# utiasDSL/upright

Hardware: AMD Instinct MI355X
Metric: batched MPC solves/sec + ms/SQP-iter, Thing 1-obj horizon=20, 1/2/4/8 GPU (higher is better)
Workload: dtype f64

## Files before the change

__graft_entry__.py:

```python
import os
import subprocess
import sys
from pathlib import Path

ROOT = Path(__file__).resolve().parent
CSRC = ROOT / "upright_amd" / "csrc"
LIB = ROOT / "upright_amd" / "libupright_mi.so"


def _newer(srcs, out):
    return (not out.exists()) or any(s.stat().st_mtime > out.stat().st_mtime for s in srcs)


def n_qp3_parts():
    import re

    m = re.search(r"#define\s+UPR_QP3_NPARTS\s+(\d+)", (CSRC / "upr_qp3_list.h").read_text())
    return int(m.group(1))


def build_engine(out=None, extra_flags=()):
    from concurrent.futures import ThreadPoolExecutor

    out = Path(out) if out else LIB
    hipcc = os.environ.get("HIPCC", "/opt/rocm/bin/hipcc")
    flags = ["--offload-arch=gfx950", "-O3", "-std=c++17", "-fPIC", "-Wno-unused-value", "-Wno-pass-failed", *extra_flags]
    obj = CSRC / "build"
    obj.mkdir(exist_ok=True)
    jobs = [([hipcc, *flags, "-c", str(CSRC / "upr_api.hip"), "-o", str(obj / "upr_api.o")], obj / "upr_api.o")]
    for k in range(n_qp3_parts()):
        o = obj / f"upr_qp3_part{k}.o"
        jobs.append(([hipcc, *flags, f"-DUPR_QP3_PART={k}", "-c", str(CSRC / "upr_qp3_inst.hip"), "-o", str(o)], o))
    with ThreadPoolExecutor(max_workers=max(1, min(len(jobs), os.cpu_count() or 1))) as ex:
        for rc, cmd in ex.map(lambda j: (subprocess.call(j[0]), j[0]), jobs):
            if rc != 0:
                raise subprocess.CalledProcessError(rc, cmd)
    subprocess.check_call([hipcc, "--offload-arch=gfx950", "-shared", "-fPIC", "-o", str(out), *[str(o) for _, o in jobs], "-lhiprtc", "-ldl"])


def build():
    srcs = sorted(CSRC.glob("*.h")) + sorted(CSRC.glob("*.hip")) + [ROOT / "include" / "upright_mi.h"]
    if _newer(srcs, LIB):
        build_engine()
    subprocess.check_call(["make", "-s", "-C", str(ROOT / "oracle")])
    emu_src = ROOT / "tests" / "emu" / "upr_emu.cpp"
    emu_out = ROOT / "tests" / "emu" / "libupr_emu.so"
    if _newer(srcs + [emu_src], emu_out):
        subprocess.check_call(["g++", "-O2", "-std=c++17", "-fPIC", "-shared", "-Wno-unknown-pragmas", "-o", str(emu_out), str(emu_src)])
    vf_src = ROOT / "tests" / "emu" / "upr_vf_emu.cpp"
    vf_out = ROOT / "tests" / "emu" / "libupr_vf_emu.so"
    if _newer(srcs + [vf_src], vf_out):
        subprocess.check_call(["g++", "-O2", "-std=c++17", "-fPIC", "-shared", "-Wno-unknown-pragmas", "-o", str(vf_out), str(vf_src)])
    sys.path.insert(0, str(ROOT))
    import upright_amd
    from upright_amd import _capi

    _capi.lib()


def smoke():
    import json

    import numpy as np

    sys.path.insert(0, str(ROOT))
    from oracle.oracle import Oracle
    from upright_amd.engine import BatchMPC
    from upright_amd.problem import thing_problem
    from upright_amd.sampling import level_tray_states, stationary_guess, waypoints_for

    arr = json.load(open(ROOT / "tests" / "golden" / "arrangements.json"))["pink_bottle"]
    P = thing_problem(arr)
    B = 4
    x0 = level_tray_states(B, seed=3)
    way = waypoints_for(P, x0)
    mpc = BatchMPC(P, B, way_p=way)
    mpc.set_observation(0.0, x0)
    mpc.advance()
    _, xs, us = mpc.solution()
    st = mpc.stats()
    xs0, us0 = stationary_guess(x0, P.N, P.nu)
    for b in range(B):
        P.way_p = way[b]
        xo, uo, so, _ = Oracle(P).solve(0.0, x0[b], xs0[b], us0[b])
        ex, eu = np.abs(xo - xs[b]).max(), np.abs(uo - us[b]).max()
        assert ex < 1e-4 and eu < 1e-4 * max(1.0, np.abs(uo).max()), (b, ex, eu)
        assert abs(np.linalg.norm(xo) - np.linalg.norm(xs[b])) < 1e-4
        assert abs(np.linalg.norm(uo) - np.linalg.norm(us[b])) < 1e-4
    print("smoke ok: qp iters", st["qp_iters_last"], "cost", st["cost"])


if __name__ == "__main__":
    build()
    if len(sys.argv) > 1 and sys.argv[1] == "smoke":
        smoke()
```

upright_amd/csrc/upr_qp3.h:

```cpp
#pragma once
#include "upr_kin.h"
#include "upr_qp.h"
#include "upr_qp2.h"

#ifndef UPR_QP3_INCEK
#define UPR_QP3_INCEK 1
#endif
#ifndef UPR_QP3_GQ
#define UPR_QP3_GQ 5
#endif
#ifndef UPR_QP3_SOFT_ROWMEM
#define UPR_QP3_SOFT_ROWMEM 1
#endif
template <int NQ_, int NB_, int NC_, int NF_, int N_, int NT_, bool ROWS_ = true, bool SOFT_ = false, bool DENSE_ = false>
struct upr_qp3_cfg {
    static constexpr int NQ = NQ_, NB = NB_, NC = NC_, NF = NF_, N = N_, NT = NT_;
    static constexpr bool ROWS = ROWS_, SOFT = SOFT_, COUPLED = DENSE_ && NB_ > 1, MULTI = NB_ > 1 && !DENSE_;
    static constexpr bool INCEK = UPR_QP3_INCEK && NB_ > 1 && !DENSE_ && NF_ == 1;
    static constexpr bool BIGF = MULTI && NF_ == 3;
    static constexpr bool KFAR = N_ > 64;
    static_assert(!KFAR || (MULTI && !BIGF && !ROWS_), "long horizons: star arrangements without friction and without state-polytopic rows (the upright_robust shape)");
    static constexpr int SB = COUPLED ? 6 * NB_ : 6, NKB = COUPLED ? N_ : N_ * NB_;
    static constexpr int NLS = COUPLED ? 36 * NB_ * NB_ : NB_ * 36;
    static constexpr int N1 = N + 1;
    static constexpr int NX = 3 * NQ, NFC = NF * NC, NU = NQ + NFC, NE = 6 * NB;
    static constexpr int NP = (NF == 3) ? 5 * NC : 0;
    static constexpr int NLF = (NF == 3) ? 9 * NC : NC;
    static constexpr int NH = NQ * (NQ + 1) / 2;
    static constexpr int NZ = N1 * NX + N * NU;
    static constexpr int NEN = 3 + 2 * NQ;
    static constexpr bool SW = NH <= 64 && 4 * NQ <= 64;
    static constexpr bool VCPRE = SW && NB_ == 1;
    static constexpr int NXI = N * NX, QX = (NXI + NT - 1) / NT;
    static constexpr int NUI = N * NU, QU = (NUI + NT - 1) / NT;
    static constexpr int NCI = N * NC, QC = (NCI + NT - 1) / NT;
    static constexpr int SS_V = 0, SS_LJI = SS_V + NQ * NX, SS_YJ = SS_LJI + NQ * NQ, SS_PB = SS_YJ + NQ, SS_STRIDE = ((SS_PB + NX + 1) & ~1);
};

#ifndef UPR_QP3_NOMAX
#define UPR_QP3_NOMAX 20
#endif
template <class C>
struct upr_qp3_far {
    static constexpr int r2(int n) { return (n + 1) & ~1; }
    static constexpr int g0 = 0, e0 = g0 + r2(C::N * C::NQ), ek = e0 + r2(C::N * C::NE), yf = ek + r2(C::N * C::NE), hf = yf + r2(C::N * C::NFC),
                         ys = hf + r2(C::N * C::NFC), zt = ys + r2(C::N * C::NE), cv = zt, nun = zt + r2(C::N * C::NE), lfi = nun + r2(C::N * C::NE),
                         Ljis = lfi + r2(C::N * C::NLF), ct = Ljis + r2(C::N * (C::SW ? C::NQ * C::NX : C::NH)),
                          cl = ct + r2(5 * C::NCI), cc = cl + r2(5 * C::NCI),
                         hee = cc + r2(5 * C::NCI), lsi = hee + r2(C::N * C::NH), Ks = lsi + r2(C::N * C::NLS),
                         cxr = Ks + r2(C::N * C::NQ * C::NX), rows = cxr + r2((C::SOFT ? 2 : 1) * (2 * C::QX + 2 * C::QU) * C::NT),
                         ot = rows + r2((C::SOFT ? 10 : 4) * (C::QX + C::QU) * C::NT), ol = ot + (C::N - 1) * UPR_QP3_NOMAX, oc = ol + (C::N - 1) * UPR_QP3_NOMAX,
                         od0 = oc + (C::N - 1) * UPR_QP3_NOMAX, heew = od0 + (C::N - 1) * UPR_QP3_NOMAX,
                         sfr = heew + r2(C::N * C::NH), sor = sfr + (C::SOFT ? 4 * r2(5 * C::NCI) : 0),
                         total = sor + ((C::SOFT && C::ROWS) ? 4 * (C::N - 1) * UPR_QP3_NOMAX : 0);
    static constexpr int sfs = r2(5 * C::NCI), sos = (C::N - 1) * UPR_QP3_NOMAX;
};

template <class C>
struct upr_qp3_lds {
    static constexpr int r2(int n) { return (n + 1) & ~1; }
    static constexpr bool KF = C::KFAR;
    static constexpr int Z = 0, S = Z + r2(C::NZ), gxs = S + r2(C::NZ), wx = gxs + r2(C::N1 * C::NX), gus = wx + r2(C::N1 * C::NX),
                         wu = gus + r2(C::N * C::NU), cs = wu + r2(C::N * C::NU), hf = cs + r2(C::N * C::NX), ys = hf + r2(C::BIGF ? 0 : C::N * C::NFC),
                         zt = ys + r2(C::N * C::NE), cv = zt, ek = zt + r2(C::N * C::NE),
                         dek = ek + r2(C::BIGF ? 0 : C::N * C::NE),
                         kend = dek + r2(C::INCEK ? C::N * C::NE : 0),
                         xlb = KF ? 0 : kend, xub = xlb + r2(C::NX), ulb = xub + r2(C::NX), uub = ulb + r2(C::NU), qd = uub + r2(C::NU),
                         rd = qd + r2(C::NX), xd = rd + r2(C::NU), erow = xd + r2(C::NX), df = erow + r2(3 * (C::NP > 0 ? C::NP : 1)),
                         Pa = df + r2(C::BIGF ? 6 * C::NFC : C::NE * C::NFC), Pb = Pa + r2(C::NX * C::NX), hux = Pb + r2(C::NX * C::NX),
                         vm = hux + r2(C::NQ * C::NX), lk = vm + 2 * r2(C::NQ * C::NX),
                         hjj = lk + 2 * r2(C::NH), vc = hjj + r2(C::NQ * C::NQ), ck = vc + r2(C::NE * C::NX),
                         VCS = (C::NE * 2 % 64 == 32 || C::NE * 2 % 64 == 0) ? C::NE + 2 : C::NE ,
                         VCN = VCS * C::NX, KS = (r2(C::NZ) / VCN < C::N - 1) ? r2(C::NZ) / VCN : C::N - 1, HXS = (C::NQ + 1) & ~1,
                         sw0 = C::VCPRE ? Pa + (C::N - 1 - KS) * VCN : Pa, sw_vcb = sw0 ,
                         sw_hj = C::VCPRE ? sw0 : sw0 + 2 * VCN, sw_hx = sw_hj + r2(C::NH), sw_pb = sw_hx + (C::NX + C::NQ) * HXS , sw_w = sw_pb + C::NX * HXS ,
                         sw_pq = sw_w + r2(C::NX) ,
                         sw_end = sw_pq + (C::VCPRE ? 0 : 2 * 9 * 64),
                         scr_sweep = ck + r2(C::NE * C::NX), scr_sw = C::SW ? ((KF || sw_end > sw0 + C::NKB * (C::SB * (C::SB + 1) / 2)) ? sw_end : sw0 + r2(C::NKB * (C::SB * (C::SB + 1) / 2))) : 0,
                         sst = (C::MULTI || C::COUPLED) ? hux : (Pa + r2(C::N * C::NE * C::NFC) > hux ? Pa + r2(C::N * C::NE * C::NFC) : hux),
                         scr_prep = sst + r2((C::MULTI || C::COUPLED) ? 0 : C::N * C::NE * C::NE), scr_rows = hux + (C::ROWS ? 2 * (C::N - 1) * UPR_QP3_NOMAX : 0),
                         scr_a = scr_sweep > scr_sw ? scr_sweep : scr_sw, scr_b = scr_prep > scr_rows ? scr_prep : scr_rows,
                         yN = scr_a > scr_b ? scr_a : scr_b, dyN = yN + r2(C::NEN),
                         eN = dyN + r2(C::NEN), jN = eN + r2(C::NEN), red = jN + r2(3 * C::NQ), RSET = (4 * (C::NT / 64) > 16 ? 4 * (C::NT / 64) : 16) , misc = red + 2 * RSET,
                         prf = misc + 16, lsik = prf + 4 * 16,    heek = lsik + r2(C::NLS), lend = heek + 2 * r2(C::NH), Pbs = KF ? kend : lend, kffs = Pbs + r2(C::N * C::NX),
                         bks = kffs + r2(C::N * C::NQ), gee = bks + r2(C::N * C::NX),
                         kend2 = gee + r2(C::N * C::NQ), clist = KF ? lend : kend2, ccnt = clist + r2(C::NB > 1 ? C::NB * C::NC : 0),
                         sdn = ccnt + r2(C::NB > 1 ? C::NB : 0),
                         plist = sdn + r2(C::COUPLED ? C::N * (C::SB * (C::SB + 1) / 2) : 0), pcnt = plist + r2(C::COUPLED ? (C::NB * (C::NB + 1) / 2) * C::NC : 0),
                         total = pcnt + r2(C::COUPLED ? C::NB * (C::NB + 1) / 2 : 0),
                         zst = KF ? kend2 : Pa, pin = KF ? zst + r2(C::N * C::NFC * 6) : Pa, ktotal = KF ? pin + r2(C::N1 * C::NX) : 0;
};

template <class C>
struct upr_qp3_ws {
    static constexpr int dx = 0, du = C::N1 * C::NX;
    static constexpr int a0 = (C::NZ + 1) & ~1;
    static constexpr int pi = a0, pin = pi + C::N1 * C::NX + (C::N1 * C::NX & 1), nu = pin + C::N1 * C::NX + (C::N1 * C::NX & 1),
                         store = nu + ((C::N * C::NE + 1) & ~1), far = store , kfar = far + upr_qp3_far<C>::total , total = ((kfar + upr_qp3_lds<C>::ktotal + 15) & ~15);
};

#ifndef UPR_QP3_KSTAGES
#define UPR_QP3_KSTAGES 6
#endif
#ifndef UPR_QP3_PRIO
#define UPR_QP3_PRIO 1
#endif
#ifndef UPR_QP3_PRIO_W0
#define UPR_QP3_PRIO_W0 3
#endif
#ifndef UPR_QP3_PRIO_VEC
#define UPR_QP3_PRIO_VEC 3
#endif
#ifndef UPR_QP3_PRIO_FWD
#define UPR_QP3_PRIO_FWD 3
#endif
#ifndef UPR_QP3_PRIO_W1
#define UPR_QP3_PRIO_W1 (C::SOFT ? 3 : 1)
#endif
#ifndef UPR_QP3_OCC1
#define UPR_QP3_OCC1 2
#endif
#ifndef UPR_QP3_PREC_MAX
#define UPR_QP3_PREC_MAX 4
#endif
#ifndef UPR_QP3_PREV_MAX
#define UPR_QP3_PREV_MAX 8
#endif
#if defined(UPR_HOST_EMU) || !UPR_QP3_PRIO
#define UPR_SETPRIO(p) ((void)0)
#else
#define UPR_SETPRIO(p) __builtin_amdgcn_s_setprio(p)
#endif
template <class C>
#define UPR_FORT(i, n) for (int i = tid(); i < (n); i += stride())

struct upr_qp3 {
    typedef upr_qp3_lds<C> O;
    typedef upr_qp3_ws<C> W;
    typedef upr_qp3_far<C> F;
    static constexpr int NQ = C::NQ, NX = C::NX, NU = C::NU, NE = C::NE, NFC = C::NFC, NC = C::NC, NF = C::NF, N = C::N, N1 = C::N1, NT = C::NT;
#ifndef UPR_HOST_EMU
    static constexpr bool SW2 = C::SW;
    static_assert(!C::SW || NT >= 128, "the two-wave matrix sweep needs two waves");
#else
    static constexpr bool SW2 = false;
#endif
    UPR_HDI static void sync_lds() { if (C::KFAR) { UPR_SYNC(); } else { UPR_SYNC_LDS(); } }
    UPR_HDI static void wsync_lds() { if (C::KFAR) { UPR_WSYNC(); } else { UPR_WSYNC_LDS(); } }
    upr_ctx ctx;
    int wb;
    UPR_HDI int lane() const {
#ifdef UPR_HOST_EMU
        return ctx.tid;
#else
        int z; asm volatile("s_mov_b32 %0, 0" : "=s"(z));
        return (int)__builtin_amdgcn_mbcnt_hi(~0u, __builtin_amdgcn_mbcnt_lo(~0u, (unsigned)z));
#endif
    }
    UPR_HDI int tid() const {
#ifdef UPR_HOST_EMU
        return ctx.tid;
#else
        return wb + lane();
#endif
    }
    UPR_HDI bool wave0() const {
#ifdef UPR_HOST_EMU
        return ctx.tid < 64;
#else
        return wb == 0;
#endif
    }
    UPR_HDI int stride() const {
// ... 1451 lines not shown
    UPR_HDI void backward_mat() {
#ifndef UPR_HOST_EMU
        static_assert(C::SW, "device instantiations run the two-wave matrix sweep (chains of up to nine joints)");
        backward_mat_sw2();
#else
#include "upr_qp3_emu_mat.h"
#endif
    }

    UPR_HDI double* Wk(int k) const { return LK + O::S + (k + 1) * NX; }
    UPR_HDI void backward_vec(bool fused = false) {
        const double irho = 1.0 / UPR_QP_RHO_N;
        if (!fused) {
        terminal_residual();
        UPR_SYNC();
        }
        toc(11);
        if (!fused && wave0()) {
            UPR_SETPRIO(UPR_QP3_PRIO_VEC);
            UPR_FORT(i, NX) {
                double v = LK[O::gxs + N * NX + i];
                if (neN > 0) {
                    if (i < NQ) { for (int q = 0; q < 3; ++q) v -= L[O::jN + q * NQ + i] * (L[O::yN + q] + irho * L[O::eN + q]); }
                    else v += L[O::yN + 3 + (i - NQ)] + irho * L[O::eN + 3 + (i - NQ)];
                }
                Wk(N - 1)[i] = v + LK[O::Pbs + (N - 1) * NX + i];
            }
            UPR_WSYNC();
#ifndef UPR_HOST_EMU
            static_assert(4 * NQ <= 64, "one quad per joint");
            {
                const int l = lane();
                const bool act = ((l & 3) < 3) && ((l >> 2) < NQ);
                const int j = act ? (l >> 2) : 0, b = act ? (l & 3) : 0;
                const int i = b * NQ + j;
                double kc[UPR_QP3_KSTAGES][NQ];
#define UPR_LOADKC(dst, kk) do { if (act && (kk) >= 1) { _Pragma("unroll") for (int m = 0; m < NQ; ++m) dst[m] = G[F::Ks + (kk) * NQ * NX + m * NX + i]; } } while (0)
#define UPR_LOADST(gk, pk, uk, kk) do { if ((kk) >= 1) { gk = LK[O::gxs + (kk) * NX + i] + LK[O::cs + (kk) * NX + i]; pk = LK[O::Pbs + ((kk) - 1) * NX + i]; uk = LK[O::gus + (kk) * NU + j]; } } while (0)
#define UPR_VECSTEP(kcx, gk, pk, uk, kk) do { \
                    double rq = cbq * wv; \
                    rq += upr_dpp_quad<0xB1>(rq); rq += upr_dpp_quad<0x4E>(rq); \
                    rq += uk; \
                    const double w0 = upr_dpp_quad<0x00>(wv), w1 = upr_dpp_quad<0x55>(wv), w2 = upr_dpp_quad<0xAA>(wv); \
                    double v0 = gk + ca0 * w0, v1 = ca1 * w1, v2 = ca2 * w2; \
                    _Pragma("unroll") for (int m = 0; m < NQ; m += 3) { \
                        v0 -= kcx[m] * upr_readlane(rq, 4 * m); \
                        if (m + 1 < NQ) v1 -= kcx[m + 1] * upr_readlane(rq, 4 * (m + 1)); \
                        if (m + 2 < NQ) v2 -= kcx[m + 2] * upr_readlane(rq, 4 * (m + 2)); } \
                    wv = ((v0 + v1) + v2) + pk; \
                    if (act) Wk((kk) - 1)[i] = wv; } while (0)
                const double ca0 = coefA(0, b), ca1 = (b >= 1) ? coefA(1, b) : 0.0, ca2 = (b >= 2) ? 1.0 : 0.0;
                const double cbq = act ? coefB(b) : 0.0;
#pragma unroll
                for (int st = 0; st < UPR_QP3_KSTAGES; ++st) {
#pragma unroll
                    for (int m = 0; m < NQ; ++m) kc[st][m] = 0.0;
                    UPR_LOADKC(kc[st], N - 1 - st);
                }
                double wv = Wk(N - 1)[i];
                double gs[2] = {0.0, 0.0}, ps[2] = {0.0, 0.0}, us2[2] = {0.0, 0.0};
                UPR_LOADST(gs[(N - 1) & 1], ps[(N - 1) & 1], us2[(N - 1) & 1], N - 1);
                constexpr int UG = C::KFAR ? UPR_QP3_KSTAGES : N - 1;
                static_assert(!C::KFAR || UPR_QP3_KSTAGES % 2 == 0, "the two operand slots keep their parity over a group");
#pragma unroll 1
                for (int k0 = N - 1; k0 >= 1; k0 -= UG) {
#pragma unroll
                    for (int sg = 0; sg < UG; ++sg) {
                        const int k = k0 - sg;
                        if (k >= 1) {
                            UPR_LOADST(gs[(N - sg) & 1], ps[(N - sg) & 1], us2[(N - sg) & 1], k - 1);
                            UPR_VECSTEP(kc[sg % UPR_QP3_KSTAGES], gs[(N - 1 - sg) & 1], ps[(N - 1 - sg) & 1], us2[(N - 1 - sg) & 1], k);
                            UPR_LOADKC(kc[sg % UPR_QP3_KSTAGES], k - UPR_QP3_KSTAGES);
                        }
                    }
                }
#undef UPR_LOADKC
#undef UPR_LOADST
#undef UPR_VECSTEP
            }
#else
            for (int k = N - 1; k >= 1; --k) {
                const double* w = Wk(k);
                UPR_FORT(i, NX) {
                    const int b = i / NQ, j = i % NQ;
                    double v = LK[O::gxs + k * NX + i] + LK[O::cs + k * NX + i];
                    for (int a = 0; a <= b; ++a) v += coefA(a, b) * w[a * NQ + j];
                    for (int m = 0; m < NQ; ++m) v -= G[F::Ks + k * NQ * NX + m * NX + i] * (LK[O::gus + k * NU + m] + h3 * w[m] + h2 * w[NQ + m] + h * w[2 * NQ + m]);
                    Wk(k - 1)[i] = v + LK[O::Pbs + (k - 1) * NX + i];
                }
            }
#endif
            UPR_SETPRIO(0);
        }
#ifndef UPR_HOST_EMU
        constexpr bool KFFW1 = SW2 && N <= 64 && NT >= 128;
        const bool kfw = KFFW1 && !fused;
        double liP[KFFW1 ? NQ : 1][KFFW1 ? NQ : 1];
        if (kfw && wb == 64) {
            const int k = (lane() < N) ? lane() : 0;
            const double* Li = G + F::Ljis + k * NQ * NX;
#pragma unroll
            for (int i = 0; i < NQ; ++i)
#pragma unroll
                for (int m = 0; m <= i; ++m) liP[i % (KFFW1 ? NQ : 1)][m % (KFFW1 ? NQ : 1)] = Li[i * NX + m];
        }
#endif
        UPR_SYNC();
        toc(10);
#ifndef UPR_HOST_EMU
        if constexpr (SW2) {
            for (int k = kfw ? tid() - 64 : tid(); k >= 0 && k < N; k += kfw ? N : stride()) {
                const double* Li = G + F::Ljis + k * NQ * NX;
                const double* w = Wk(k);
                double li[NQ][NQ], tv[NQ], y[NQ];
#pragma unroll
                for (int i = 0; i < NQ; ++i)
#pragma unroll
                    for (int m = 0; m <= i; ++m) li[i][m] = kfw ? liP[i % (KFFW1 ? NQ : 1)][m % (KFFW1 ? NQ : 1)] : Li[i * NX + m];
#pragma unroll
                for (int i = 0; i < NQ; ++i) tv[i] = fused ? LK[O::kffs + k * NQ + i] : LK[O::gus + k * NU + i] + h3 * w[i] + h2 * w[NQ + i] + h * w[2 * NQ + i];
#pragma unroll
                for (int i = 0; i < NQ; ++i) { double t = 0.0;
#pragma unroll
                    for (int m = 0; m <= i; ++m) t += li[i][m] * tv[m];
                    y[i] = t; }
#pragma unroll
                for (int i = 0; i < NQ; ++i) { double t = 0.0;
#pragma unroll
                    for (int m = i; m < NQ; ++m) t += li[m][i] * y[m];
                    LK[O::kffs + k * NQ + i] = t; }
            }
        } else
#endif
        UPR_FORT(k, N) {
            const double* Lp = G + F::Ljis + k * C::NH;
            const double* w = Wk(k);
            double y[NQ], kk[NQ];
#pragma unroll
            for (int i = 0; i < NQ; ++i) { double t = LK[O::gus + k * NU + i] + h3 * w[i] + h2 * w[NQ + i] + h * w[2 * NQ + i];
#pragma unroll
                for (int m = 0; m < i; ++m) t -= Lp[i * (i + 1) / 2 + m] * y[m];
                y[i] = t * Lp[i * (i + 1) / 2 + i]; }
#pragma unroll
            for (int i = NQ - 1; i >= 0; --i) { double t = y[i];
#pragma unroll
                for (int m = i + 1; m < NQ; ++m) t -= Lp[m * (m + 1) / 2 + i] * kk[m];
                kk[i] = t * Lp[i * (i + 1) / 2 + i]; }
#pragma unroll
            for (int i = 0; i < NQ; ++i) LK[O::kffs + k * NQ + i] = kk[i];
        }
        UPR_SYNC();
    }

    template <bool COST>
    UPR_HDI void forward() {
#ifndef UPR_HOST_EMU
        constexpr int NTL = NT - 64, CH = (NX + 3) / 4, QV = (N * NE * 4 + NTL - 1) / NTL, QCT = (C::NCI + NTL - 1) / NTL;
        static_assert((C::KFAR || C::NKB <= NTL) && NTL % 4 == 0, "tail lanes: one per Schur block (KFAR: a loop over the blocks)");
        const int tl = tid() - 64;
        constexpr int QCS = (N * NX + NTL - 1) / NTL;
        constexpr int QH = (N * NQ + NTL - 1) / NTL;
        constexpr bool PRE_V = QV <= UPR_QP3_PREV_MAX, PRE_K = QCS * NE <= 24;
        constexpr int SB = C::SB;
        constexpr bool DIST = SB > 6;
        double ckq[PRE_V ? QV : 1][CH], lsr[DIST ? 1 : SB * SB], bkq[QCT][NF == 3 ? 9 : 1], yfq[QCT][NF == 3 ? 3 : 1];
        double heeq[QH][NQ], ckc[PRE_K ? QCS : 1][PRE_K ? NE : 1];
#endif
        if (wave0()) {
            UPR_SETPRIO(UPR_QP3_PRIO_FWD);
            UPR_FORT(i, NX) {
                const int b = i / NQ, j = i % NQ;
                const double uj = -LK[O::kffs + j];
                Sx(0)[i] = 0.0;
                Sx(1)[i] = coefB(b) * uj + LK[O::bks + i];
                if (b == 0) Su(0)[j] = uj;
            }
            UPR_WSYNC();
#ifndef UPR_HOST_EMU
            static_assert(4 * NQ <= 64, "one quad per joint");
            {
                const int l = lane();
                const bool act = ((l & 3) < 3) && ((l >> 2) < NQ);
                const int j = act ? (l >> 2) : 0, b = act ? (l & 3) : 3;
                const int i = (act ? b : 0) * NQ + j;
                double kq[UPR_QP3_KSTAGES][NQ];
#define UPR_LOADKQ(dst, kk) do { if (act && (kk) < N) { _Pragma("unroll") for (int c = 0; c < NQ; ++c) dst[c] = G[F::Ks + (kk) * NQ * NX + j * NX + b * NQ + c]; } } while (0)
#define UPR_LOADST(bk, fk, kk) do { if ((kk) < N) { bk = LK[O::bks + (kk) * NX + i]; fk = LK[O::kffs + (kk) * NQ + j]; } } while (0)
#define UPR_FWDSTEP(kqx, bk, fk, kk) do { \
                    double xs[NQ]; \
                    _Pragma("unroll") for (int c = 0; c < NQ; ++c) xs[c] = upr_bpermute(xv, src + 16 * c); \
                    __builtin_amdgcn_sched_barrier(0);    \
                    double d0 = (b == 0) ? fk : 0.0, d1 = 0.0, d2 = 0.0; \
                    _Pragma("unroll") for (int c = 0; c < NQ; c += 3) { \
                        d0 += kqx[c] * xs[c]; \
                        if (c + 1 < NQ) d1 += kqx[c + 1] * xs[c + 1]; \
                        if (c + 2 < NQ) d2 += kqx[c + 2] * xs[c + 2]; } \
                    double d = (d0 + d1) + d2;    \
                    d += upr_dpp_quad<0xB1>(d); d += upr_dpp_quad<0x4E>(d); \
                    const double x0 = upr_dpp_quad<0x00>(xv), x1 = upr_dpp_quad<0x55>(xv), x2 = upr_dpp_quad<0xAA>(xv); \
                    xv = ((bk + ra0 * x0) + (ra1 * x1 + ra2 * x2)) - cb * d; \
                    if (act) { Sx((kk) + 1)[i] = xv; if (b == 0) Su(kk)[j] = -d; } } while (0)
                const double ra0 = (b == 0) ? 1.0 : 0.0, ra1 = (b == 0) ? h : ((b == 1) ? 1.0 : 0.0), ra2 = (b == 0) ? h2 : ((b == 1) ? h : ((b == 2) ? 1.0 : 0.0));
                const double cb = act ? coefB(b) : 0.0;
                const int src = 4 * (l & 3);
#pragma unroll
                for (int st = 0; st < UPR_QP3_KSTAGES; ++st) {
#pragma unroll
                    for (int c = 0; c < NQ; ++c) kq[st][c] = 0.0;
                    UPR_LOADKQ(kq[st], 1 + st);
                }
                double xv = Sx(1)[i];
                double bs[2] = {0.0, 0.0}, fs[2] = {0.0, 0.0};
                UPR_LOADST(bs[1], fs[1], 1);
                constexpr int UG = C::KFAR ? UPR_QP3_KSTAGES : N - 1;
#pragma unroll 1
                for (int k0 = 1; k0 < N; k0 += UG) {
#pragma unroll
                    for (int sg = 0; sg < UG; ++sg) {
                        const int k = k0 + sg;
                        if (k < N) {
                            UPR_LOADST(bs[(sg + 2) & 1], fs[(sg + 2) & 1], k + 1);
                            UPR_FWDSTEP(kq[sg % UPR_QP3_KSTAGES], bs[(sg + 1) & 1], fs[(sg + 1) & 1], k);
                            UPR_LOADKQ(kq[sg % UPR_QP3_KSTAGES], k + UPR_QP3_KSTAGES);
                        }
                    }
                }
#undef UPR_LOADKQ
#undef UPR_LOADST
#undef UPR_FWDSTEP
            }
#else
            for (int k = 1; k < N; ++k) {
                const double* sx = Sx(k);
                UPR_FORT(i, NX) {
                    const int b = i / NQ, j = i % NQ;
                    const double* Kr = G + F::Ks + k * NQ * NX + j * NX;
                    double d0 = LK[O::kffs + k * NQ + j], d1 = 0.0, d2 = 0.0;
                    for (int c = 0; c < NQ; ++c) { d0 += Kr[c] * sx[c]; d1 += Kr[NQ + c] * sx[NQ + c]; d2 += Kr[2 * NQ + c] * sx[2 * NQ + c]; }
                    const double uj = -(d0 + d1 + d2);
                    double r = coefB(b) * uj + LK[O::bks + k * NX + i];
                    for (int a = b; a < 3; ++a) r += coefA(b, a) * sx[a * NQ + j];
                    Sx(k + 1)[i] = r;
                    if (b == 0) Su(k)[j] = uj;
                }
            }
#endif
            UPR_SETPRIO(0);
#ifndef UPR_HOST_EMU
            if (!ROWMEM) load_rows();
#endif
        }
#ifndef UPR_HOST_EMU
        else {
            if (!ROWMEM) load_rows();
            if (PRE_V) {
#pragma unroll
                for (int q = 0; q < QV; ++q) {
                    const int e4 = tl + q * NTL;
                    if (e4 < N * NE * 4) {
                        const int e = e4 >> 2, part = e4 & 3;
                        const double* Ck = rec(e / NE) + lin_gx + (e % NE) * NX + part * CH;
#pragma unroll
                        for (int c = 0; c < CH; ++c) ckq[q % (PRE_V ? QV : 1)][c] = (part * CH + c < NX) ? Ck[c] : 0.0;
                    }
                }
            }
            if (!DIST && !C::KFAR && tl < C::NKB) {
#pragma unroll
                for (int r = 0; r < SB; ++r)
#pragma unroll
                    for (int m = 0; m <= r; ++m) lsr[r * SB + m] = G[F::lsi + tl * SB * SB + r * SB + m];
            }
            if (COST) {
#pragma unroll
                for (int q = 0; q < QH; ++q) {
                    const int e = tl + q * NTL;
                    if (e < N * NQ) {
                        const int k = e / NQ, i = e % NQ;
#pragma unroll
                        for (int j = 0; j < NQ; ++j) heeq[q][j] = G[hee_w + k * C::NH + upr_tri(NQ, i, j)];
                    }
                }
                if (PRE_K) {
#pragma unroll
                    for (int q = 0; q < QCS; ++q) {
                        const int e = tl + q * NTL;
                        if (e < N * NX) {
                            const double* Ck = rec(e / NX) + lin_gx + e % NX;
#pragma unroll
                            for (int r = 0; r < NE; ++r) ckc[q % (PRE_K ? QCS : 1)][r % (PRE_K ? NE : 1)] = Ck[r * NX];
                        }
                    }
                }
            }
#pragma unroll
            for (int q = 0; q < QCT; ++q) {
                const int ic = tl + q * NTL;
                if (ic < C::NCI) {
                    const int k = ic / NC, ci = ic % NC;
                    if (NF == 3) {
#pragma unroll
                        for (int a = 0; a < 9; ++a) bkq[q][a] = G[F::lfi + k * C::NLF + 9 * ci + a];
#pragma unroll
                        for (int a = 0; a < 3; ++a) yfq[q][a] = G[F::yf + k * NFC + 3 * ci + a];
                    } else { bkq[q][0] = G[F::lfi + k * C::NLF + ci]; yfq[q][0] = G[F::yf + k * NFC + ci]; }
                }
            }
        }
#endif
        ftoc(6, 5);
        UPR_SYNC();
        toc(12);
#ifndef UPR_HOST_EMU
        if (PRE_V) {
#pragma unroll
            for (int q = 0; q < QV; ++q) {
                const int e4 = tl + q * NTL;
                const bool act = tl >= 0 && e4 < N * NE * 4;
                const int e = act ? (e4 >> 2) : 0, part = e4 & 3;
                double v = 0.0;
                {
                    const double* sx = Sx(e / NE) + part * CH;
                    double sv[CH];
#pragma unroll
                    for (int c = 0; c < CH; ++c) sv[c] = sx[c];
#pragma unroll
                    for (int c = 0; c < CH; ++c) v += (act ? ckq[q % (PRE_V ? QV : 1)][c] : 0.0) * sv[c];
                }
                v += upr_dpp_quad<0xB1>(v); v += upr_dpp_quad<0x4E>(v);
                if (act && part == 0) { LK[O::cv + e] = v; if (C::INCEK && COST) LK[O::dek + e] = v; }
            }
        } else {
            constexpr int GQ = UPR_QP3_GQ;
#pragma unroll 1
            for (int q0 = 0; q0 < QV; q0 += GQ) {
                double cb[GQ][CH];
#pragma unroll
                for (int g = 0; g < GQ; ++g) {
                    const int e4 = tl + (q0 + g) * NTL;
                    const bool act = tl >= 0 && (q0 + g < QV) && e4 < N * NE * 4;
                    const int e = act ? (e4 >> 2) : 0, part = e4 & 3;
                    const double* Ck = rec(e / NE) + lin_gx + (e % NE) * NX + part * CH;
#pragma unroll
                    for (int c = 0; c < CH; ++c) cb[g][c] = (act && part * CH + c < NX) ? Ck[c] : 0.0;
                }
#pragma unroll
                for (int g = 0; g < GQ; ++g) {
                    const int e4 = tl + (q0 + g) * NTL;
                    const bool act = tl >= 0 && (q0 + g < QV) && e4 < N * NE * 4;
                    const int e = act ? (e4 >> 2) : 0, part = e4 & 3;
                    const double* sx = Sx(e / NE) + part * CH;
                    double v = 0.0;
#pragma unroll
                    for (int c = 0; c < CH; ++c) v += cb[g][c] * ((part * CH + c < NX) ? sx[c] : 0.0);
                    v += upr_dpp_quad<0xB1>(v); v += upr_dpp_quad<0x4E>(v);
                    if (act && part == 0) { LK[O::cv + e] = v; if (C::INCEK && COST) LK[O::dek + e] = v; }
                }
            }
        }
        if (COST) {
#pragma unroll
            for (int q = 0; q < QH; ++q) {
                const int e = tl + q * NTL;
                if (tl >= 0 && e < N * NQ) {
                    const double* sx = Sx(e / NQ);
                    double v = 0.0;
#pragma unroll
                    for (int j = 0; j < NQ; ++j) v += heeq[q][j] * sx[j];
                    LK[O::gee + e] = h * v;
                }
            }
        }
        sync_lds();
        if (DIST) {
            constexpr int NROW = C::NKB * SB, QD = (NROW + NTL - 1) / NTL;
            double tv1[QD];
#pragma unroll
            for (int pass = 0; pass < 2; ++pass) {
#pragma unroll
                for (int q = 0; q < QD; ++q) {
                    const int e = tl + q * NTL;
                    if (tl >= 0 && e < NROW) {
                        const int kb = e / SB, r = e % SB;
                        const double* Ls = G + F::lsi + kb * SB * SB;
                        double lv[SB], xv[SB];
#pragma unroll
                        for (int m = 0; m < SB; ++m) { lv[m] = (pass == 0) ? Ls[r * SB + m] : Ls[m * SB + r]; xv[m] = LK[O::cv + kb * SB + m]; }
                        double v = (pass == 0) ? LK[O::ys + e] : 0.0;
#pragma unroll
                        for (int m = 0; m < SB; ++m) v += (((pass == 0) ? (m <= r) : (m >= r)) ? lv[m] : 0.0) * xv[m];
                        tv1[q] = v;
                    }
                }
                sync_lds();
#pragma unroll
                for (int q = 0; q < QD; ++q) {
                    const int e = tl + q * NTL;
                    if (tl >= 0 && e < NROW) { LK[O::cv + e] = tv1[q]; if (pass == 1) G[F::nun + e] = tv1[q]; }
                }
                if (pass == 0) sync_lds();
            }
        } else
        for (int kb = tl; kb >= 0 && kb < C::NKB; kb += NTL) {
            if (C::KFAR) {
#pragma unroll
                for (int r = 0; r < SB; ++r)
#pragma unroll
                    for (int m = 0; m <= r; ++m) lsr[r * SB + m] = G[F::lsi + kb * SB * SB + r * SB + m];
            }
            double cvr[SB], t1[SB];
#pragma unroll
            for (int r = 0; r < SB; ++r) cvr[r] = LK[O::cv + kb * SB + r];
#pragma unroll
            for (int r = 0; r < SB; ++r) { double v = LK[O::ys + kb * SB + r];
#pragma unroll
                for (int m = 0; m <= r; ++m) v += lsr[r * SB + m] * cvr[m];
                t1[r] = v; }
#pragma unroll
            for (int r = 0; r < SB; ++r) { double v = 0.0;
#pragma unroll
                for (int m = r; m < SB; ++m) v += lsr[m * SB + r] * t1[m];
                LK[O::cv + kb * SB + r] = v; G[F::nun + kb * SB + r] = v; }
        }
        sync_lds();
#pragma unroll
        for (int q = 0; q < QCT; ++q) {
            const int ic = tl + q * NTL;
            if (tl >= 0 && ic < C::NCI) {
                const int k = ic / NC, ci = ic % NC;
                if (NF == 3) {
                    double dfn[3], tf[3];
                    const int rb = (C::NB > 1) ? 6 * P->contact_body2[ci] : 0;
#pragma unroll
                    for (int a = 0; a < 3; ++a) { double v = 0.0;
#pragma unroll
                        for (int r = 0; r < 6; ++r) v += DF(rb + r, 3 * ci + a) * LK[O::cv + k * NE + rb + r];
                        dfn[a] = v; }
                    if (C::COUPLED && P->contact_body1[ci] >= 0) {
                        const int rb1 = 6 * P->contact_body1[ci];
#pragma unroll
                        for (int a = 0; a < 3; ++a)
#pragma unroll
                            for (int r = 0; r < 6; ++r) dfn[a] += L[O::df + (rb1 + r) * NFC + 3 * ci + a] * LK[O::cv + k * NE + rb1 + r];
                    }
#pragma unroll
                    for (int a = 0; a < 3; ++a) { double v = yfq[q][a];
#pragma unroll
                        for (int b2 = 0; b2 <= a; ++b2) v += bkq[q][3 * a + b2] * dfn[b2];
                        tf[a] = v; }
#pragma unroll
                    for (int a = 0; a < 3; ++a) { double v = 0.0;
#pragma unroll
                        for (int b2 = a; b2 < 3; ++b2) v += bkq[q][3 * b2 + a] * tf[b2];
                        Su(k)[NQ + 3 * ci + a] = -v; }
                } else {
                    double dfn = 0.0;
                    const int rb = (C::NB > 1) ? 6 * P->contact_body2[ci] : 0;
#pragma unroll
                    for (int r = 0; r < 6; ++r) dfn += L[O::df + (rb + r) * NFC + ci] * LK[O::cv + k * NE + rb + r];
                    if (C::COUPLED && P->contact_body1[ci] >= 0) {
                        const int rb1 = 6 * P->contact_body1[ci];
#pragma unroll
                        for (int r = 0; r < 6; ++r) dfn += L[O::df + (rb1 + r) * NFC + ci] * LK[O::cv + k * NE + rb1 + r];
                    }
                    const double lf = bkq[q][0];
                    Su(k)[NQ + ci] = -lf * (yfq[q][0] + lf * dfn);
                }
            }
        }
#else
        UPR_FORT(e, N * NE) {
            const int k = e / NE, r = e % NE;
            const double* Ck = rec(k) + lin_gx + r * NX; const double* sx = Sx(k);
            double v = 0.0;
            for (int c = 0; c < NX; ++c) v += Ck[c] * sx[c];
            LK[O::cv + e] = v;
            if (C::INCEK && COST) LK[O::dek + e] = v;
        }
        UPR_SYNC();
        UPR_FORT(kb, C::NKB) {
            constexpr int SB = C::SB;
            const double* Ls = G + F::lsi + kb * SB * SB;
            double t1[SB];
#pragma unroll
            for (int r = 0; r < SB; ++r) { double v = LK[O::ys + kb * SB + r];
#pragma unroll
                for (int m = 0; m <= r; ++m) v += Ls[r * SB + m] * LK[O::cv + kb * SB + m];
                t1[r] = v; }
#pragma unroll
            for (int r = 0; r < SB; ++r) { double v = 0.0;
#pragma unroll
                for (int m = r; m < SB; ++m) v += Ls[m * SB + r] * t1[m];
                LK[O::cv + kb * SB + r] = v; G[F::nun + kb * SB + r] = v; }
        }
        UPR_SYNC();
        for (int q = 0; q < C::QC; ++q) {
            const int ic = tid() + q * NT;
            if (ic < C::NCI) {
                const int k = ic / NC, ci = ic % NC;
                if (NF == 3) {
                    double dfn[3], tf[3];
                    for (int a = 0; a < 3; ++a) { double v = 0.0;
                        if (C::BIGF) { const int rb = 6 * P->contact_body2[ci]; for (int r = 0; r < 6; ++r) v += DF(rb + r, 3 * ci + a) * G[F::nun + k * NE + rb + r]; }
                        else for (int r = 0; r < NE; ++r) v += L[O::df + r * NFC + 3 * ci + a] * G[F::nun + k * NE + r];
                        dfn[a] = v; }
                    const double* Bk = G + F::lfi + k * C::NLF + 9 * ci;
                    for (int a = 0; a < 3; ++a) { double v = G[F::yf + k * NFC + 3 * ci + a]; for (int b2 = 0; b2 <= a; ++b2) v += Bk[3 * a + b2] * dfn[b2]; tf[a] = v; }
                    for (int a = 0; a < 3; ++a) { double v = 0.0; for (int b2 = a; b2 < 3; ++b2) v += Bk[3 * b2 + a] * tf[b2]; Su(k)[NQ + 3 * ci + a] = -v; }
                } else {
                    double dfn = 0.0;
                    for (int r = 0; r < NE; ++r) dfn += L[O::df + r * NFC + ci] * G[F::nun + k * NE + r];
                    const double lf = G[F::lfi + k * C::NLF + ci];
                    Su(k)[NQ + ci] = -lf * (G[F::yf + k * NFC + ci] + lf * dfn);
                }
            }
        }
#endif
        if (neN > 0) UPR_FORT(q, C::NEN) {
            double v;
            if (q < 3) { v = L[O::eN + q]; for (int j = 0; j < NQ; ++j) v -= L[O::jN + q * NQ + j] * Sx(N)[j]; }
            else v = L[O::eN + q] + Sx(N)[NQ + (q - 3)];
            L[O::dyN + q] = v / UPR_QP_RHO_N;
        }
#ifndef UPR_HOST_EMU
        sync_lds();
        if (COST) {
            double* pin = LK + O::pin;
#pragma unroll
            for (int q = 0; q < QCS; ++q) {
                const int e = tl + q * NTL;
                if (tl >= 0 && e < N * NX) {
                    const int k = e / NX, i = e % NX;
                    const double sxi = Sx(k)[i];
                    double v = LK[O::gxs + e] + LK[O::wx + e] * sxi + h * L[O::qd + i] * sxi;
                    if (i < NQ) v += LK[O::gee + k * NQ + i];
                    if (PRE_K) {
#pragma unroll
                        for (int r = 0; r < NE; ++r) v += ckc[q % (PRE_K ? QCS : 1)][r % (PRE_K ? NE : 1)] * LK[O::cv + k * NE + r];
                    } else {
                        const double* Ck = rec(k) + lin_gx + i;
                        double cr[NE];
#pragma unroll
                        for (int r = 0; r < NE; ++r) cr[r] = Ck[r * NX];
#pragma unroll
                        for (int r = 0; r < NE; ++r) v += cr[r] * LK[O::cv + k * NE + r];
                    }
                    pin[e] = v;
                }
            }
            if (tl < 0 && tl + 64 < NX) {
                const int i = tl + 64, e = N * NX + i;
                double v = LK[O::gxs + e] + LK[O::wx + e] * Sx(N)[i];
                if (neN > 0) {
                    if (i < NQ) { for (int q = 0; q < 3; ++q) v -= L[O::jN + q * NQ + i] * (L[O::yN + q] + L[O::dyN + q]); }
                    else v += L[O::yN + 3 + (i - NQ)] + L[O::dyN + 3 + (i - NQ)];
                }
                pin[e] = v;
            }
            sync_lds();
            costate_sums();
        }
#else
        UPR_SYNC();
        if (COST) costates();
#endif
    }

    UPR_HDI void costate_sums() {
        double* pin = LK + O::pin;
        UPR_FORT(j, NQ) {
            double pq = pin[N * NX + j], pvv = pin[N * NX + NQ + j], pa = pin[N * NX + 2 * NQ + j];
#pragma unroll
            for (int k = N - 1; k >= 1; --k) {
                const double nq_ = pin[k * NX + j] + pq;
                const double nv_ = pin[k * NX + NQ + j] + h * pq + pvv;
                const double na_ = pin[k * NX + 2 * NQ + j] + h2 * pq + h * pvv + pa;
                pq = nq_; pvv = nv_; pa = na_;
                pin[k * NX + j] = pq; pin[k * NX + NQ + j] = pvv; pin[k * NX + 2 * NQ + j] = pa;
            }
        }
        sync_lds();
    }

    UPR_HDI void costates() {
        double* pin = LK + O::pin;
        UPR_FORT(e, N1 * NX) {
            const int k = e / NX, i = e % NX;
            const double* sx = Sx(k);
            double v = LK[O::gxs + e] + LK[O::wx + e] * sx[i];
            if (k < N) {
                v += h * L[O::qd + i] * sx[i];
                if (i < NQ) for (int j = 0; j < NQ; ++j) v += h * G[hee_w + k * C::NH + upr_tri(NQ, i, j)] * sx[j];
                const double* Ck = rec(k) + lin_gx;
                for (int q = 0; q < NE; ++q) v += Ck[q * NX + i] * LK[O::cv + k * NE + q];
            } else if (neN > 0) {
                if (i < NQ) { for (int q = 0; q < 3; ++q) v -= L[O::jN + q * NQ + i] * (L[O::yN + q] + L[O::dyN + q]); }
                else v += L[O::yN + 3 + (i - NQ)] + L[O::dyN + 3 + (i - NQ)];
            }
            pin[e] = v;
        }
        UPR_SYNC();
        costate_sums();
    }

    UPR_HDI void sweep_row(int what, double alpha, double c, double ds, double& t, double& lam, double cterm, double& acc, double* aux) const {
        const double rp = c - t;
        if (what == 3) { const double a = fabs(rp); if (a > acc) acc = a; *aux += lam * t; return; }
        const double dt = ds + rp;
        const double rc = (mode == 0) ? lam * t : lam * t + cterm;
        const double rt = upr_rcp(t);
        const double dl = -(rc + lam * dt) * rt;
        if (what == 0) {
            acc = fmax(acc, fmax(-dt * rt, -dl * upr_rcp(lam)));
            if (aux) *aux += dt * dl;
        }
        else if (what == 5) { const double v = (lam + alpha * dl) * (t + alpha * dt); acc = fmin(acc, v); *aux += v; }
        else { t += alpha * dt; lam += alpha * dl; }
    }
    UPR_HDI void sweep_row_soft(int what, double alpha, double c, double ds, double& t, double& lam, double& sig, double& tau, double& gam,
                                double Zp, double zp, double cterm, double cterm_s, double& acc, double* aux) {
        const double rp = c + sig - t, rps = sig - tau;
        if (what == 3) {
            const double a = fmax(fabs(rp), fabs(rps)); if (a > acc) acc = a;
            *aux += lam * t + gam * tau;
            soft_stat = fmax(soft_stat, fabs(Zp * sig + zp - lam - gam));
            return;
        }
        const double rc = (mode == 0) ? lam * t : lam * t + cterm, rcs = (mode == 0) ? gam * tau : gam * tau + cterm_s;
        const double rt = upr_rcp(t), rtau = upr_rcp(tau);
        const double w0 = lam * rt, ws_ = gam * rtau, rD = upr_rcp(Zp + w0 + ws_);
        const double a = (Zp * sig + zp - lam - gam) + (rc + lam * rp) * rt + (rcs + gam * rps) * rtau;
        const double dsg = -(a + w0 * ds) * rD;
        const double dt = ds + rp + dsg, dtau = dsg + rps;
        const double dl = -(rc + lam * dt) * rt, dg = -(rcs + gam * dtau) * rtau;
        if (what == 0) { acc = fmax(fmax(acc, fmax(-dt * rt, -dl * upr_rcp(lam))), fmax(-dtau * rtau, -dg * upr_rcp(gam))); if (aux) *aux += dt * dl + dtau * dg; }
        else if (what == 5) { const double v = (lam + alpha * dl) * (t + alpha * dt), vs = (gam + alpha * dg) * (tau + alpha * dtau); acc = fmin(acc, fmin(v, vs)); *aux += v + vs; }
        else { t += alpha * dt; lam += alpha * dl; sig += alpha * dsg; tau += alpha * dtau; gam += alpha * dg; }
    }
    UPR_HDI double ineq_sweep(int what, double alpha, double* aux, const double (&ctm)[NCTR], bool reload = true) {
        ftoc(10, 4);
        if (ROWMEM && reload) load_rows();
        double acc = (what == 5) ? 1e300 : 0.0;
        const int tid_ = tid();
        constexpr int NR5 = 5 * C::NCI, QR5 = (NR5 + NT - 1) / NT, QS5 = C::SOFT ? QR5 : 1;
        double tv[QR5], lv[QR5], cv5[QR5], ssv[QS5][4];
        auto fetch_fr = [&]() {
#pragma unroll
            for (int q = 0; q < QR5; ++q) {
                const int e = tid_ + q * NT, ec = (e < NR5) ? e : 0;
                tv[q] = G[F::ct + ec]; lv[q] = G[F::cl + ec]; cv5[q] = G[F::cc + ec];
                if (C::SOFT && softp) {
#pragma unroll
                    for (int u = 0; u < 4; ++u) ssv[q % QS5][u] = G[F::sfr + u * F::sfs + ec];
                }
            }
        };
        constexpr int QOS = (C::SOFT && C::ROWS) ? QO : 1;
        double gq[QO][NQ], od[QO], otv[QO], olv[QO], ocv[QO], osv[QOS][4];
        auto fetch_or = [&]() {
#pragma unroll
            for (int q = 0; q < QO; ++q) {
                const int e = tid_ + q * NT, ec = (e < (N - 1) * no) ? e : 0;
                const int k = 1 + ec / no, r = ec % no, ei = (k - 1) * UPR_QP3_NOMAX + r;
                const double* g = orow(k, r);
#pragma unroll
                for (int i = 0; i < NQ; ++i) gq[q][i] = g[i];
                od[q] = G[F::od0 + ei]; otv[q] = G[F::ot + ei]; olv[q] = G[F::ol + ei]; ocv[q] = G[F::oc + ei];
                if (C::SOFT && C::ROWS && softp) {
#pragma unroll
                    for (int u = 0; u < 4; ++u) osv[q % QOS][u] = G[F::sor + u * F::sos + ei];
                }
            }
        };
        const bool w4 = what == 4;
        const int wstep = w4 ? 2 : what;
        auto tgt = [&](int i) -> double { return C::KFAR ? ((ctm[0] != 0.0) ? G[F::cxr + i * NT + tid_] : 0.0) : ctm[i % NCTR]; };
        auto hard = [&](double c, double ds, double cn, double& t, double& lam, double ct) {
            if (!w4) { sweep_row(what, alpha, c, ds, t, lam, ct, acc, aux); return; }
            double unused = 0.0;
            sweep_row(2, alpha, c, ds, t, lam, ct, unused, nullptr);
            sweep_row(3, 0.0, cn, 0.0, t, lam, 0.0, acc, aux);
        };
        auto soft = [&](double c, double ds, double cn, double& t, double& lam, double& sg, double& ta, double& ga, double Zp, double zp, double ct, double cts) {
            if (!w4) { sweep_row_soft(what, alpha, c, ds, t, lam, sg, ta, ga, Zp, zp, ct, cts, acc, aux); return; }
            double unused = 0.0;
            sweep_row_soft(2, alpha, c, ds, t, lam, sg, ta, ga, Zp, zp, ct, cts, unused, nullptr);
            sweep_row_soft(3, 0.0, cn, 0.0, t, lam, sg, ta, ga, Zp, zp, 0.0, 0.0, acc, aux);
        };
#pragma unroll (C::KFAR ? 1 : C::QX)
        for (int q = 0; q < C::QX; ++q) {
            const int ix = tid_ + q * NT;
            if (ix < C::NXI) {
                const int zo = NX + ix, i = ix % NX;
                ldx(q);
                const double X = LK[O::Z + zo], dS = LK[O::S + zo];
                const double Xn = w4 ? upr_step(X, alpha, dS) : X;
                if (C::SOFT && softx) {
                    soft(X - L[O::xlb + i], dS, Xn - L[O::xlb + i], tx[q % QXR][0], lx[q % QXR][0], sgx[q % QXS][0], tax[q % QXS][0], gax[q % QXS][0], ZL, zL, tgt(2 * q), tgt(NCT0 + 2 * q));
                    soft(L[O::xub + i] - X, -dS, L[O::xub + i] - Xn, tx[q % QXR][1], lx[q % QXR][1], sgx[q % QXS][1], tax[q % QXS][1], gax[q % QXS][1], ZU, zU, tgt(2 * q + 1), tgt(NCT0 + 2 * q + 1));
                } else {
                    hard(X - L[O::xlb + i], dS, Xn - L[O::xlb + i], tx[q % QXR][0], lx[q % QXR][0], tgt(2 * q));
                    hard(L[O::xub + i] - X, -dS, L[O::xub + i] - Xn, tx[q % QXR][1], lx[q % QXR][1], tgt(2 * q + 1));
                }
                if (wstep == 2) stx(q);
            }
        }
ftoc(6, 4);
#pragma unroll (C::KFAR ? 1 : C::QU)
        for (int q = 0; q < C::QU; ++q) {
            const int iu = tid() + q * NT;
            if (iu < C::NUI) {
                const int i = iu % NU;
// ... 687 lines not shown
```

Measured before the change: 545,400.

## Pipeline per-knot trailing work behind wave 0's forward rollout via hand-overs

Adds a TRAIL path for single-body 256-thread configs in which the three trailing waves process groups of knots (constraint products, Schur solve, friction updates, costate inputs) as soon as wave 0's forward rollout passes each hand-over point, instead of waiting for the full rollout. Wave 0 inserts LDS barriers at the group boundaries, and the old bulk post-rollout tail loops are disabled. This overlaps tail computation with the serial forward sweep, at the cost of extra barriers inside the rollout and one wave 0 stalling at the hand-overs. A host emulator build for the new path is also added.

Result: slower. 531,100 (-2.6%).

```diff
diff --git a/__graft_entry__.py b/__graft_entry__.py
--- a/__graft_entry__.py
+++ b/__graft_entry__.py
@@ -51,6 +51,10 @@
     vf_out = ROOT / "tests" / "emu" / "libupr_vf_emu.so"
     if _newer(srcs + [vf_src], vf_out):
         subprocess.check_call(["g++", "-O2", "-std=c++17", "-fPIC", "-shared", "-Wno-unknown-pragmas", "-o", str(vf_out), str(vf_src)])
+    tr_src = ROOT / "tests" / "emu_trail" / "upr_trail_emu.cpp"
+    tr_out = ROOT / "tests" / "emu_trail" / "libupr_trail_emu.so"
+    if _newer(srcs + [tr_src], tr_out):
+        subprocess.check_call(["g++", "-O2", "-std=c++17", "-fPIC", "-shared", "-Wno-unknown-pragmas", "-o", str(tr_out), str(tr_src)])
     sys.path.insert(0, str(ROOT))
     import upright_amd
     from upright_amd import _capi
diff --git a/upright_amd/csrc/upr_qp3.h b/upright_amd/csrc/upr_qp3.h
--- a/upright_amd/csrc/upr_qp3.h
+++ b/upright_amd/csrc/upr_qp3.h
@@ -12,6 +12,12 @@
 #ifndef UPR_QP3_SOFT_ROWMEM
 #define UPR_QP3_SOFT_ROWMEM 1
 #endif
+#ifndef UPR_QP3_TRAIL
+#define UPR_QP3_TRAIL 1
+#endif
+#ifndef UPR_QP3_TRAIL_G
+#define UPR_QP3_TRAIL_G 6
+#endif
 template <int NQ_, int NB_, int NC_, int NF_, int N_, int NT_, bool ROWS_ = true, bool SOFT_ = false, bool DENSE_ = false>
 struct upr_qp3_cfg {
     static constexpr int NQ = NQ_, NB = NB_, NC = NC_, NF = NF_, N = N_, NT = NT_;
@@ -19,6 +25,7 @@
     static constexpr bool INCEK = UPR_QP3_INCEK && NB_ > 1 && !DENSE_ && NF_ == 1;
     static constexpr bool BIGF = MULTI && NF_ == 3;
     static constexpr bool KFAR = N_ > 64;
+    static constexpr bool TRAIL = UPR_QP3_TRAIL && NB_ == 1 && NT_ == 256 && N_ >= 2 && N_ <= 64 && 3 * NQ_ <= 32 && NC_ <= 32;
     static_assert(!KFAR || (MULTI && !BIGF && !ROWS_), "long horizons: star arrangements without friction and without state-polytopic rows (the upright_robust shape)");
     static constexpr int SB = COUPLED ? 6 * NB_ : 6, NKB = COUPLED ? N_ : N_ * NB_;
     static constexpr int NLS = COUPLED ? 36 * NB_ * NB_ : NB_ * 36;
@@ -1776,6 +1783,12 @@
         UPR_SYNC();
     }
 
+    static constexpr int TRAIL_G = UPR_QP3_TRAIL_G, TRAIL_NHO = 1 + (N - 2 + TRAIL_G - 1) / TRAIL_G;
+    static_assert(TRAIL_G >= 1 && TRAIL_G <= 6, "a group is at most two knots for each of the three trailing waves");
+    static constexpr bool trail_ho(int k) { return (k % TRAIL_G == 0 && k < N - 2) || k == N - 2; }
+    static constexpr int trail_count() { int c = 0; for (int k = 1; k < N; ++k) c += trail_ho(k) ? 1 : 0; return c; }
+    static constexpr int trail_end(int hd) { return ((hd * TRAIL_G < N - 2) ? hd * TRAIL_G : N - 2) + 2; }
+
     template <bool COST>
     UPR_HDI void forward() {
 #ifndef UPR_HOST_EMU
@@ -1802,6 +1815,7 @@
             UPR_WSYNC();
 #ifndef UPR_HOST_EMU
             static_assert(4 * NQ <= 64, "one quad per joint");
+            if (C::TRAIL) UPR_SYNC_LDS();
             {
                 const int l = lane();
                 const bool act = ((l & 3) < 3) && ((l >> 2) < NQ);
@@ -1845,6 +1859,7 @@
                         if (k < N) {
                             UPR_LOADST(bs[(sg + 2) & 1], fs[(sg + 2) & 1], k + 1);
                             UPR_FWDSTEP(kq[sg % UPR_QP3_KSTAGES], bs[(sg + 1) & 1], fs[(sg + 1) & 1], k);
+                            if (C::TRAIL && trail_ho(1 + sg)) UPR_SYNC_LDS();
                             UPR_LOADKQ(kq[sg % UPR_QP3_KSTAGES], k + UPR_QP3_KSTAGES);
                         }
                     }
@@ -1875,6 +1890,122 @@
 #endif
         }
 #ifndef UPR_HOST_EMU
+        else if (C::TRAIL) {
+            static_assert(!C::TRAIL || (trail_count() == TRAIL_NHO - 1 && trail_end(TRAIL_NHO - 1) == N), "wave 0 and the trailing waves meet at the same hand-overs");
+            static_assert(!C::TRAIL || (4 * NE <= 32 && NX <= 32 && NC <= 32 && SB == 6 && !DIST), "the jobs of a knot fit half a wave");
+            const int tw = (wb >> 6) - 1, hh = lane() >> 5, hl = lane() & 31;
+            const int row = hl >> 2, part = hl & 3;
+            constexpr int SL = 4 * NE;
+            double ckt[CH], lst[SB * SB], bkt[NF == 3 ? 9 : 1], yft[NF == 3 ? 3 : 1], het[NQ], cct[NE];
+#pragma unroll 1
+            for (int hd = 0; hd < TRAIL_NHO; ++hd) {
+                const int ka = (hd == 0) ? 0 : trail_end(hd - 1), kb = trail_end(hd);
+                const bool on = ka + tw + 3 * hh < kb;
+                const int k = on ? ka + tw + 3 * hh : ka;
+                if (on && hl < 4 * NE) {
+                    const double* Ck = rec(k) + lin_gx + row * NX + part * CH;
+#pragma unroll
+                    for (int c = 0; c < CH; ++c) ckt[c] = (part * CH + c < NX) ? Ck[c] : 0.0;
+                }
+                if (on && hl == SL) {
+#pragma unroll
+                    for (int r = 0; r < SB; ++r)
+#pragma unroll
+                        for (int m = 0; m <= r; ++m) lst[r * SB + m] = G[F::lsi + k * SB * SB + r * SB + m];
+                }
+                if (on && hl < NC) {
+                    if (NF == 3) {
+#pragma unroll
+                        for (int a = 0; a < 9; ++a) bkt[a] = G[F::lfi + k * C::NLF + 9 * hl + a];
+#pragma unroll
+                        for (int a = 0; a < 3; ++a) yft[a] = G[F::yf + k * NFC + 3 * hl + a];
+                    } else { bkt[0] = G[F::lfi + k * C::NLF + hl]; yft[0] = G[F::yf + k * NFC + hl]; }
+                }
+                if (COST && on && hl < NQ) {
+#pragma unroll
+                    for (int j = 0; j < NQ; ++j) het[j] = G[hee_w + k * C::NH + upr_tri(NQ, hl, j)];
+                }
+                if (COST && on && hl < NX) {
+                    const double* Ck = rec(k) + lin_gx + hl;
+#pragma unroll
+                    for (int r = 0; r < NE; ++r) cct[r] = Ck[r * NX];
+                }
+                UPR_SYNC_LDS();
+                {
+                    const bool act = on && hl < 4 * NE;
+                    const double* sx = Sx(k) + part * CH;
+                    double sv[CH];
+#pragma unroll
+                    for (int c = 0; c < CH; ++c) sv[c] = sx[c];
+                    double v = 0.0;
+#pragma unroll
+                    for (int c = 0; c < CH; ++c) v += (act ? ckt[c] : 0.0) * ((part * CH + c < NX) ? sv[c] : 0.0);
+                    v += upr_dpp_quad<0xB1>(v); v += upr_dpp_quad<0x4E>(v);
+                    if (act && part == 0) LK[O::cv + k * NE + row] = v;
+                }
+                if (COST && on && hl < NQ) {
+                    const double* sx = Sx(k);
+                    double v = 0.0;
+#pragma unroll
+                    for (int j = 0; j < NQ; ++j) v += het[j] * sx[j];
+                    LK[O::gee + k * NQ + hl] = h * v;
+                }
+                wsync_lds();
+                if (on && hl == SL) {
+                    double cvr[SB], t1[SB];
+#pragma unroll
+                    for (int r = 0; r < SB; ++r) cvr[r] = LK[O::cv + k * SB + r];
+#pragma unroll
+                    for (int r = 0; r < SB; ++r) { double v = LK[O::ys + k * SB + r];
+#pragma unroll
+                        for (int m = 0; m <= r; ++m) v += lst[r * SB + m] * cvr[m];
+                        t1[r] = v; }
+#pragma unroll
+                    for (int r = 0; r < SB; ++r) { double v = 0.0;
+#pragma unroll
+                        for (int m = r; m < SB; ++m) v += lst[m * SB + r] * t1[m];
+                        LK[O::cv + k * SB + r] = v; G[F::nun + k * SB + r] = v; }
+                }
+                wsync_lds();
+                if (on && hl < NC) {
+                    const int ci = hl;
+                    if (NF == 3) {
+                        double dfn[3], tf[3];
+#pragma unroll
+                        for (int a = 0; a < 3; ++a) { double v = 0.0;
+#pragma unroll
+                            for (int r = 0; r < 6; ++r) v += DF(r, 3 * ci + a) * LK[O::cv + k * NE + r];
+                            dfn[a] = v; }
+#pragma unroll
+                        for (int a = 0; a < 3; ++a) { double v = yft[a];
+#pragma unroll
+                            for (int b2 = 0; b2 <= a; ++b2) v += bkt[3 * a + b2] * dfn[b2];
+                            tf[a] = v; }
+#pragma unroll
+                        for (int a = 0; a < 3; ++a) { double v = 0.0;
+#pragma unroll
+                            for (int b2 = a; b2 < 3; ++b2) v += bkt[3 * b2 + a] * tf[b2];
+                            Su(k)[NQ + 3 * ci + a] = -v; }
+                    } else {
+                        double dfn = 0.0;
+#pragma unroll
+                        for (int r = 0; r < 6; ++r) dfn += L[O::df + r * NFC + ci] * LK[O::cv + k * NE + r];
+                        const double lf = bkt[0];
+                        Su(k)[NQ + ci] = -lf * (yft[0] + lf * dfn);
+                    }
+                }
+                if (COST && on && hl < NX) {
+                    const int i = hl, e = k * NX + i;
+                    const double sxi = Sx(k)[i];
+                    double v = LK[O::gxs + e] + LK[O::wx + e] * sxi + h * L[O::qd + i] * sxi;
+                    if (i < NQ) v += LK[O::gee + k * NQ + i];
+#pragma unroll
+                    for (int r = 0; r < NE; ++r) v += cct[r] * LK[O::cv + k * NE + r];
+                    LK[O::pin + e] = v;
+                }
+            }
+            if (!ROWMEM) load_rows();
+        }
         else {
             if (!ROWMEM) load_rows();
             if (PRE_V) {
@@ -1936,6 +2067,7 @@
         UPR_SYNC();
         toc(12);
 #ifndef UPR_HOST_EMU
+        if (!C::TRAIL) {
         if (PRE_V) {
 #pragma unroll
             for (int q = 0; q < QV; ++q) {
@@ -2091,6 +2223,7 @@
                     Su(k)[NQ + ci] = -lf * (yfq[q][0] + lf * dfn);
                 }
             }
+        }
         }
 #else
         UPR_FORT(e, N * NE) {
@@ -2147,11 +2280,13 @@
             L[O::dyN + q] = v / UPR_QP_RHO_N;
         }
 #ifndef UPR_HOST_EMU
-        sync_lds();
+        constexpr bool W0END = C::TRAIL && COST;
+        static_assert(!W0END || (C::NEN <= 64 && NX <= 64), "the terminal step and knot N's costate terms on wave 0");
+        if (W0END) { if (wave0()) wsync_lds(); } else sync_lds();
         if (COST) {
             double* pin = LK + O::pin;
 #pragma unroll
-            for (int q = 0; q < QCS; ++q) {
+            for (int q = 0; q < (C::TRAIL ? 0 : QCS); ++q) {
                 const int e = tl + q * NTL;
                 if (tl >= 0 && e < N * NX) {
                     const int k = e / NX, i = e % NX;
@@ -2181,7 +2316,7 @@
                 }
                 pin[e] = v;
             }
-            sync_lds();
+            if (W0END) { if (wave0()) wsync_lds(); } else sync_lds();
             costate_sums();
         }
 #else
```
